# mgp25/OpenLTE

Measured on AMD Instinct MI355X. Metric: DL subframes/sec @20MHz 100RB 64QAM, full chain FFT->CE->demap->rate-unmatch->turbo(REF)->CRC (SURVEY 8d W4), higher is better.
Workload: dtype i8 IQ in, f32 FFT/CE/equaliser, i8 soft bits, i16 path metrics (differences exact modulo 2^16); 1 GPU; W4 full DL chain: 20 MHz/100 RB/64QAM, 9 allocations per subframe (8x12 PRB TBS 3240 + 1x4 PRB TBS 1064), 65536 subframes per GPU, int8 IQ in HBM; subframes_per_gpu=65536, N_ant=1, CFI=2, channel_estimate_form=compact, decoder=REF (reference-faithful, bit-exact), unique_subframes=96, streams_per_gpu=1

## Files before the change

openlte_amd/csrc/ctx.cc:

```cpp
#include <cmath>

#include <chrono>
#include <cstdlib>

#include <algorithm>

#include "ctx.hpp"
#include "build_id.h"

#include <cstring>

#include "lte_tables.h"

extern "C" {

int mi_lte_version(void) { return MI_LTE_VERSION; }
const char *mi_lte_build_id(void) { return MI_LTE_BUILD_ID; }

int mi_lte_device_count(void)
{
    int n = 0;
    if (hipGetDeviceCount(&n) != hipSuccess) return 0;
    return n;
}

int mi_lte_ctx_create(int device, mi_lte_ctx **out)
{
    if (!out) return MI_LTE_ERR_INVALID_ARG;
    *out  = nullptr;
    int n = mi_lte_device_count();
    if (n <= 0 || device < 0 || device >= n) {
        fprintf(stderr, "mi_lte: no usable HIP device %d (found %d); this library has no CPU fallback\n", device, n);
        return MI_LTE_ERR_NO_DEVICE;
    }
    mi_lte_ctx *ctx = new mi_lte_ctx();
    ctx->device     = device;
    if (const char *e = getenv("MI_LTE_NO_MERGED_DECODE")) ctx->merged_decode = atoi(e) == 0;
    hipDeviceProp_t prop;
    if (hipSetDevice(device) != hipSuccess || hipGetDeviceProperties(&prop, device) != hipSuccess) {
        delete ctx;
        return MI_LTE_ERR_HIP;
    }
    ctx->dev_name = std::string(prop.name) + " (" + prop.gcnArchName + ")";
    if (std::strncmp(prop.gcnArchName, "gfx950", 6) != 0) {
        fprintf(stderr, "mi_lte: device %d is %s, but the kernels are built for gfx950 only\n", device, prop.gcnArchName);
        delete ctx;
        return MI_LTE_ERR_NO_DEVICE;
    }
    if (hipStreamCreateWithFlags(&ctx->stream, hipStreamNonBlocking) != hipSuccess || hipEventCreate(&ctx->ev0) != hipSuccess ||
        hipEventCreate(&ctx->ev1) != hipSuccess) {
        delete ctx;
        return MI_LTE_ERR_HIP;
    }
    *out = ctx;
    return MI_LTE_OK;
}

void mi_lte_ctx_destroy(mi_lte_ctx *ctx)
{
    if (!ctx) return;
    (void)hipSetDevice(ctx->device);
    (void)hipStreamSynchronize(ctx->stream);
    if (ctx->host_cache_free) ctx->host_cache_free(ctx);
    for (void *p : ctx->owned) (void)hipFree(p);
    for (hipEvent_t e : ctx->prof_pool) (void)hipEventDestroy(e);
    if (ctx->scratch) (void)hipFree(ctx->scratch);
    if (ctx->h_small) (void)hipHostFree(ctx->h_small);
    if (ctx->h_bounce) (void)hipHostFree(ctx->h_bounce);
    for (int k = 0; k < 2; k++)
        if (ctx->ev_bounce[k]) (void)hipEventDestroy(ctx->ev_bounce[k]);
    if (ctx->h_flag) (void)hipHostFree(ctx->h_flag);
    if (ctx->ev0) (void)hipEventDestroy(ctx->ev0);
    if (ctx->ev1) (void)hipEventDestroy(ctx->ev1);
    if (ctx->stream) (void)hipStreamDestroy(ctx->stream);
    delete ctx;
}

int mi_lte_set_turbo_small_batch(mi_lte_ctx *ctx, uint32_t n_cb_max)
{
    if (!ctx) return MI_LTE_ERR_INVALID_ARG;
    ctx->siso_small_max = n_cb_max;
    return MI_LTE_OK;
}

int mi_lte_set_turbo_merged(mi_lte_ctx *ctx, uint32_t on)
{
    if (!ctx) return MI_LTE_ERR_INVALID_ARG;
    ctx->merged_decode = on != 0;
    return MI_LTE_OK;
}
// ... 498 lines not shown
```

openlte_amd/csrc/ctx.hpp:

```cpp
#pragma once

#include <hip/hip_runtime.h>

#include <cstdint>
#include <cstdio>
#include <map>
#include <string>
#include <vector>

#include "../../include/mi_lte.h"

struct TurboTables {
    uint16_t *d_pi  = nullptr;
    uint16_t *d_inv = nullptr;
    uint16_t *d_inv2 = nullptr;
    uint32_t *d_pi_row = nullptr, *d_inv_row = nullptr;
};

struct RmTables {
    uint16_t *d_tabs = nullptr;
    uint32_t *d_nnn  = nullptr;
};

enum : uint32_t { MI_FFT_TWC_P2 = 0, MI_FFT_TWC_P3 = 32, MI_FFT_TWC_L2048 = 288, MI_FFT_TWC_L1024 = 1312, MI_FFT_TWC_L256 = 1824, MI_FFT_TWC_L128 = 1952,
                  MI_FFT_TWC_X2 = 2016, MI_FFT_TWC_X3 = 2048,
                  MI_FFT_TWC_TOTAL = 2560 };

constexpr uint32_t MI_CRC_TAB_BIAS = 8;

struct mi_lte_ctx {
    int                device = -1;
    hipStream_t        stream = nullptr;
    hipEvent_t         ev0 = nullptr, ev1 = nullptr;
    std::string        err;
    std::string        dev_name;
    std::string        last_kernels;
    double             copy_rates[3] = {0, 0, 0};
    void              *scratch       = nullptr;
    size_t             scratch_bytes = 0;
    uint32_t          *h_flag = nullptr, *d_flag = nullptr;
    uint32_t           flag_seq = 0;
    uint32_t *bcjr_early_buf = nullptr; size_t bcjr_early_cap = 0;
    struct { uint32_t *chg; uint32_t n_pairs, n_iter, n_cb; } bcjr_early = {nullptr, 0, 0, 0};
    bool               bcjr_block_lds_set = false;
    uint32_t           siso_small_max = 4096;
    bool               merged_decode = true;
    void              *h_small = nullptr, *d_small = nullptr;
    void              *h_bounce = nullptr, *d_bounce = nullptr;
    hipEvent_t         ev_bounce[2] = {nullptr, nullptr};
    bool               bounce_failed = false;
    std::map<uint64_t, TurboTables> turbo_tables;
    std::map<uint32_t, RmTables>    rm_tables;
    std::vector<void *> owned;

    uint32_t *d_gold_x1 = nullptr, *d_gold_x2b = nullptr;
    uint32_t  gold_words = 0;
    void     *d_pusch_shapes = nullptr;

    float2   *d_fft_tw  = nullptr;
    uint32_t *d_crc_tab = nullptr;
    float2   *d_prach_tab = nullptr;
    float2   *d_prach_tab4 = nullptr;

    bool                                   prof_on = false, prof_armed = false;
    std::vector<hipEvent_t>                prof_pool;
    size_t                                 prof_used = 0;
    std::vector<std::pair<const char *, size_t>> prof_recs;
    std::string                            prof_report;

    void *host_cache = nullptr;
    void (*host_cache_free)(mi_lte_ctx *) = nullptr;
};

void mi_prof_begin(mi_lte_ctx *ctx, const char *name);
void mi_prof_end(mi_lte_ctx *ctx);

#define MI_LAUNCH(ctx, name, kernel, grid, block, shmem, ...)                                         \
    do {                                                                                             \
        mi_prof_begin((ctx), (name));                                                                \
        hipLaunchKernelGGL(kernel, grid, block, shmem, (ctx)->stream, __VA_ARGS__);                  \
        mi_prof_end((ctx));                                                                          \
    } while (0)

#define MI_HIP_CHECK(ctx, call)                                                                      \
    do {                                                                                             \
        hipError_t e_ = (call);                                                                      \
        if (e_ != hipSuccess) {                                                                      \
            (ctx)->err = std::string(#call) + ": " + hipGetErrorString(e_);                          \
            return MI_LTE_ERR_HIP;                                                                   \
        }                                                                                            \
    } while (0)

#define MI_H2D(ctx, d, h, n) do { const int rc_ = mi_lte_memcpy_h2d((ctx), (d), (h), (n)); if (rc_ != MI_LTE_OK) return rc_; } while (0)
#define MI_D2H(ctx, h, d, n) do { const int rc_ = mi_lte_memcpy_d2h((ctx), (h), (d), (n)); if (rc_ != MI_LTE_OK) return rc_; } while (0)

template <typename F> struct OnFail {
    F    f;
    bool armed = true;
    ~OnFail() { if (armed) f(); }
// ... 53 lines not shown
```

openlte_amd/csrc/turbo.hip:

```cpp
#include <algorithm>
#include <cstring>
#include <type_traits>
#include <vector>

#include "plan_core.hpp"

namespace {

constexpr uint32_t RX_NULL_AS_INT = 10000;

__host__ __device__ inline uint32_t kpad64(uint32_t K) { return (K + 63u) & ~63u; }


__device__ __forceinline__ int sbyte(uint32_t w, int k) { return (int)__builtin_amdgcn_sbfe(w, 8 * k, 8); }

typedef __attribute__((address_space(3))) const uint8_t  lds_u8_t;
typedef __attribute__((address_space(3))) const int8_t   lds_i8_t;
typedef __attribute__((address_space(3))) const uint16_t lds_u16_t;
__device__ __forceinline__ uint32_t lds_u8(uint32_t addr) { return *(lds_u8_t *)(uintptr_t)addr; }
__device__ __forceinline__ int      lds_i8(uint32_t addr) { return *(lds_i8_t *)(uintptr_t)addr; }
__device__ __forceinline__ uint32_t lds_u16(uint32_t addr) { return *(lds_u16_t *)(uintptr_t)addr; }

typedef short v2s __attribute__((ext_vector_type(2)));
__device__ __forceinline__ v2s      as_v2s(uint32_t w) { return __builtin_bit_cast(v2s, w); }
__device__ __forceinline__ uint32_t as_u32(v2s v) { return __builtin_bit_cast(uint32_t, v); }
__device__ __forceinline__ v2s      even2(uint32_t w) { return (as_v2s(w) << 8) >> 8; }
__device__ __forceinline__ v2s      odd2(uint32_t w) { return as_v2s(w) >> 8; }
__device__ __forceinline__ uint32_t merge_bytes(v2s e, v2s o) { return __builtin_amdgcn_perm(as_u32(o), as_u32(e), 0x06020400u); }
__device__ __forceinline__ v2s      abs2(v2s a) { return __builtin_elementwise_max(a, (v2s)(0) - a); }
__device__ __forceinline__ uint32_t neg_mask(v2s d)
{
    uint32_t m;
    asm("v_pk_ashrrev_i16 %0, 15, %1 op_sel_hi:[0,1]" : "=v"(m) : "v"(as_u32(d)));
    return m;
}
__device__ __forceinline__ v2s bit_select(uint32_t m, v2s yes, v2s no) { return as_v2s((as_u32(yes) & m) | (as_u32(no) & ~m)); }
__device__ __forceinline__ v2s half_sum(v2s a, v2s b)
{
    uint32_t t = as_u32(a + b);
    asm("" : "+v"(t));
    return as_v2s(t) >> 1;
}

__device__ __forceinline__ int soft_xor(int a, int b)
{
    int mag = (abs(a) + abs(b)) >> 1;
    return ((a < 0) != (b < 0)) ? -mag : mag;
}


template <typename Op> __device__ __forceinline__ int wave_reduce_i(int v, Op op)
{
    v = op(v, __builtin_amdgcn_update_dpp(v, v, 0xB1, 0xF, 0xF, false));
    v = op(v, __builtin_amdgcn_update_dpp(v, v, 0x4E, 0xF, 0xF, false));
    v = op(v, __builtin_amdgcn_update_dpp(v, v, 0x141, 0xF, 0xF, false));
    v = op(v, __builtin_amdgcn_update_dpp(v, v, 0x140, 0xF, 0xF, false));
    return op(op(__builtin_amdgcn_readlane(v, 0), __builtin_amdgcn_readlane(v, 16)), op(__builtin_amdgcn_readlane(v, 32), __builtin_amdgcn_readlane(v, 48)));
}
__device__ __forceinline__ int      wave_max_i(int v) { return wave_reduce_i(v, [](int a, int b) { return max(a, b); }); }
__device__ __forceinline__ uint32_t wave_xor_u(uint32_t v) { return (uint32_t)wave_reduce_i((int)v, [](int a, int b) { return a ^ b; }); }
__device__ __forceinline__ float    wave_max_f(float v)
{
    return __int_as_float(wave_max_i(__float_as_int(v)));
}

__device__ __forceinline__ float block_max_abs_f(float v, float *red )
{
    v = wave_max_f(v);
    __syncthreads();
    if ((threadIdx.x & 63) == 0) red[threadIdx.x >> 6] = v;
    __syncthreads();
    float r = red[0];
    for (uint32_t w = 1; w < (blockDim.x >> 6); w++) r = fmaxf(r, red[w]);
    return r;
// ... 352 lines not shown
    __device__ __forceinline__ void load16_pk(uint32_t u, int nvalid, uint32_t (&vp)[3][8], uint32_t e_lds, bool in_lds) const
    {
        auto emit = [&](int x, const int (&acc)[16]) {
#pragma unroll
            for (int j = 0; j < 8; j++) vp[x][j] = __builtin_amdgcn_perm((uint32_t)acc[2 * j + 1], (uint32_t)acc[2 * j], 0x05040100u);
        };
        if (in_lds) gather16_staged(e_lds, u, nvalid, emit);
        else        gather16(e, u, nvalid, emit);
    }
    __device__ __forceinline__ bool window_ok() const { return Nnn + 48 <= e_cap; }
    __device__ __forceinline__ void gather_windowed_pk(uint32_t u, int nvalid, uint32_t (&vp)[3][8], int8_t *lds, uint32_t el) const
    {
        uint4 *l = reinterpret_cast<uint4 *>(lds);
        for (uint32_t base = 0; base < E; base += Nnn) {
            const uint32_t len = min(Nnn, E - base), shift = base & 15u, end = shift + len, nq = end >> 4, tail = end & 15u;
            const uint4   *gp = reinterpret_cast<const uint4 *>(e + (base - shift));
            RankWords rw;
            load_ranks(u, nvalid, rw);
            if (base) __syncthreads();
#pragma unroll 4
            for (uint32_t w = threadIdx.x; w < nq; w += blockDim.x) l[w] = gp[w];
            if (threadIdx.x == (nq & 63u)) {
                uint4 t = make_uint4(0, 0, 0, 0);
                if (tail) {
                    t = gp[nq];
                    uint32_t c[4] = {t.x, t.y, t.z, t.w};
#pragma unroll
                    for (uint32_t k = 0; k < 4; k++) {
                        const int keep = (int)tail - 4 * (int)k;
                        c[k] = keep >= 4 ? c[k] : keep <= 0 ? 0u : (c[k] & ((1u << (8 * keep)) - 1u));
                    }
                    t = make_uint4(c[0], c[1], c[2], c[3]);
                }
                l[nq] = t;
            }
            __syncthreads();
            if (nvalid > 0) {
#pragma unroll
                for (int x = 0; x < 3; x++) {
                    const uint32_t w[8] = {rw.raw[x][0].x, rw.raw[x][0].y, rw.raw[x][0].z, rw.raw[x][0].w, rw.raw[x][1].x, rw.raw[x][1].y, rw.raw[x][1].z, rw.raw[x][1].w};
                    int acc[16];
#pragma unroll
                    for (int k = 0; k < 16; k++) {
                        const uint32_t r = (k & 1) ? (w[k >> 1] >> 16) : (w[k >> 1] & 0xFFFFu);
                        acc[k] = lds_i8(el + shift + min(r, len));
                    }
#pragma unroll
                    for (int j = 0; j < 8; j++)
                        vp[x][j] = as_u32(as_v2s(vp[x][j]) + as_v2s(__builtin_amdgcn_perm((uint32_t)acc[2 * j + 1], (uint32_t)acc[2 * j], 0x05040100u)));
                }
            }
        }
    }
};
__device__ __forceinline__ void SrcRateUnmatch::seg(const_seg_fwd_t &sg)
{
    tabs = (const uint16_t *)sg.tabs; nnn = (const uint32_t *)sg.nnn; g.desc += sg.cb_base;
}
struct SrcRateUnmatchPk : SrcRateUnmatch { static constexpr bool kPacked = true; };

constexpr uint32_t QTAB_N = 4096;
constexpr uint32_t QTAB_HALF = 2048;
constexpr uint32_t MTAB_N = 256;
constexpr uint32_t PREP_RED_AT = 2 * MTAB_N, PREP_E_AT = PREP_RED_AT + 64, PREP_QTAB_AT = PREP_E_AT, PREP_Q0_AT = PREP_QTAB_AT + QTAB_N;
__host__ __device__ constexpr uint32_t prep_lds_bytes(uint32_t Kp, uint32_t e_cap) { return PREP_E_AT + (e_cap > QTAB_N + Kp ? e_cap : QTAB_N + Kp); }

__device__ __forceinline__ uint32_t pack4u(uint32_t b0, uint32_t b1, uint32_t b2, uint32_t b3) { return b0 | (b1 << 8) | (b2 << 16) | (b3 << 24); }
__device__ __forceinline__ uint32_t bias4(uint32_t w) { return w ^ 0x80808080u; }
template <int K4> __device__ __forceinline__ uint32_t abs_sum2(uint32_t wa_biased, uint32_t wb_biased)
{
    return __builtin_amdgcn_msad_u8(wb_biased, 0x80u << (8 * K4), __builtin_amdgcn_msad_u8(wa_biased, 0x80u << (8 * K4), 0u));
}
__device__ __forceinline__ void abs_sum16(const uint4 &A, const uint4 &B, uint32_t (&w)[16], uint32_t &wmax)
{
    const uint32_t a[4] = {bias4(A.x), bias4(A.y), bias4(A.z), bias4(A.w)}, b[4] = {bias4(B.x), bias4(B.y), bias4(B.z), bias4(B.w)};
#pragma unroll
    for (int j = 0; j < 4; j++) {
        w[4 * j]     = abs_sum2<0>(a[j], b[j]);
        w[4 * j + 1] = abs_sum2<1>(a[j], b[j]);
        w[4 * j + 2] = abs_sum2<2>(a[j], b[j]);
        w[4 * j + 3] = abs_sum2<3>(a[j], b[j]);
        wmax = max(max(wmax, w[4 * j]), max(w[4 * j + 1], max(w[4 * j + 2], w[4 * j + 3])));
    }
}
__device__ __forceinline__ uint4 lookup16(uint32_t base, const uint32_t (&w)[16])
{
    uint32_t o[4];
#pragma unroll
    for (int j = 0; j < 4; j++) o[j] = pack4u(lds_u8(base + w[4 * j]), lds_u8(base + w[4 * j + 1]), lds_u8(base + w[4 * j + 2]), lds_u8(base + w[4 * j + 3]));
    return make_uint4(o[0], o[1], o[2], o[3]);
}
__device__ __forceinline__ uint4 gather16_bytes(uint32_t base, const uint32_t (&idx)[16]) { return lookup16(base, idx); }

template <typename Src, int NSLOT, bool MULTI = false>
#ifndef PREP_WPE
#define PREP_WPE 6
#endif
#ifndef PREP_WPE_PK
#define PREP_WPE_PK 6
#endif
__global__ __launch_bounds__(384) __attribute__((amdgpu_waves_per_eu(Src::kPacked ? PREP_WPE_PK : PREP_WPE, 8))) void k_turbo_prep(Src src, uint32_t K_arg, uint32_t n_cb_arg,
                                                    const uint16_t *__restrict__ pi_arg, PrepOut out, MultiArgs ma)
{
    static_assert(NSLOT == 1, "one unit per thread (K <= 6144 -> at most 384 units)");
    uint32_t K = K_arg, n_cb = n_cb_arg, bidx = blockIdx.x;
    size_t   seg_off = 0;
    const uint16_t *__restrict__ pi = pi_arg;
    if constexpr (MULTI) {
        const_seg_t &sg = multi_seg(ma, blockIdx.x >> 9);
        K = sg.K; n_cb = sg.n_cb; pi = (const uint16_t *)sg.pi; bidx = blockIdx.x - sg.wg_cb; seg_off = sg.arr_off;
        src.e_cap = sg.e_cap;
        src.seg(sg);
    }
    extern __shared__ __attribute__((aligned(16))) int8_t sm[];
    const uint32_t cb = xcd_cb(bidx, n_cb), tile = cb >> 6, lane = cb & 63, Kp = kpad64(K), n_units = Kp >> 4;
    const size_t   tile_off = seg_off + (size_t)tile * Kp * 64;
    if (cb >= n_cb) {
        if (MULTI && cb < ((n_cb + 63u) & ~63u) && threadIdx.x < n_units)
#pragma unroll
            for (int a = 0; a < 6; a++) *reinterpret_cast<uint4 *>(out.arr[a] + unit_off(tile_off, lane, threadIdx.x)) = make_uint4(0, 0, 0, 0);
        return;
    }
    int8_t        *qtab = sm + PREP_QTAB_AT, *qc = qtab + QTAB_HALF, *mtab1 = sm, *mtab2 = mtab1 + MTAB_N, *e_lds = sm + PREP_E_AT;
    int8_t        *q0_lds = sm + PREP_Q0_AT;
    float         *red_f  = reinterpret_cast<float *>(sm + PREP_RED_AT);
    int           *red_i  = reinterpret_cast<int *>(sm + PREP_RED_AT);
    src.init(cb, K);
    const uint32_t u  = threadIdx.x;
    const int      nv = (u < n_units) ? min(16, max(0, (int)K - 16 * (int)u)) : -1;
    const bool     e_in_lds = src.stage_e(e_lds);

    typedef typename std::conditional<Src::kIntPath, int, float>::type val_t;
    val_t    v[Src::kPacked ? 1 : 3][16];
    uint32_t vp[3][8];
    float    mx;
    int      mxi = 0;
    if constexpr (Src::kPacked) {
#pragma unroll
        for (int x = 0; x < 3; x++)
#pragma unroll
            for (int j = 0; j < 8; j++) vp[x][j] = 0;
        if (!e_in_lds && src.window_ok()) src.gather_windowed_pk(u, nv, vp, e_lds, PREP_E_AT);
        else if (nv > 0) src.load16_pk(u, nv, vp, PREP_E_AT, e_in_lds);
        v2s hi = (v2s)(0), lo = (v2s)(0);
#pragma unroll
        for (int x = 0; x < 3; x++)
#pragma unroll
            for (int j = 0; j < 8; j++) { hi = __builtin_elementwise_max(hi, as_v2s(vp[x][j])); lo = __builtin_elementwise_min(lo, as_v2s(vp[x][j])); }
        mxi = block_max_i(max(max((int)hi.x, (int)hi.y), -min((int)lo.x, (int)lo.y)), red_i);
        mx  = (float)mxi;
    } else {
        if (nv > 0) src.load16(u, nv, v, PREP_E_AT, e_in_lds);
        else {
#pragma unroll
            for (int x = 0; x < 3; x++)
#pragma unroll
                for (int k = 0; k < 16; k++) v[Src::kPacked ? 0 : x][k] = 0;
        }
        if constexpr (Src::kIntPath) {
            int hi = 0, lo = 0;
#pragma unroll
            for (int x = 0; x < 3; x++)
#pragma unroll
                for (int k = 0; k < 16; k += 2) { hi = max(max(hi, v[Src::kPacked ? 0 : x][k]), v[x][k + 1]); lo = min(min(lo, v[Src::kPacked ? 0 : x][k]), v[x][k + 1]); }
            mxi = block_max_i(max(hi, -lo), red_i);
            mx  = (float)mxi;
        } else {
            float mxv = 0;
#pragma unroll
            for (int x = 0; x < 3; x++)
#pragma unroll
                for (int k = 0; k < 16; k++) mxv = fmaxf(mxv, fabsf(v[Src::kPacked ? 0 : x][k]));
            mx = block_max_abs_f(mxv, red_f);
        }
    }
    const bool use_qtab = Src::kIntegerValued && mx < (float)QTAB_HALF;
    const bool identity = Src::kIntPath && mxi == 127;
    const bool halving = Src::kPacked && mxi == 254;
    if (use_qtab && !identity && !halving) {
        if constexpr (Src::kIntPath) {
            for (int d = (int)threadIdx.x - mxi; d <= mxi; d += (int)blockDim.x) qc[d] = (int8_t)(int)((float)d * 127.0f / mx);
        } else {
            for (uint32_t a = threadIdx.x; a <= (uint32_t)mx; a += blockDim.x) qtab[a] = (int8_t)(int)((float)a * 127.0f / mx);
        }
        __syncthreads();
    }

    uint4 Q[3];
#pragma unroll
    for (int x = 0; x < 3; x++) {
        if constexpr (Src::kPacked) {
            uint32_t o[4];
            if (identity) {
#pragma unroll
                for (int j = 0; j < 4; j++) o[j] = __builtin_amdgcn_perm(vp[x][2 * j + 1], vp[x][2 * j], 0x06040200u);
            } else if (halving) {
#pragma unroll
                for (int j = 0; j < 4; j++) {
                    const v2s a = as_v2s(vp[x][2 * j]), b = as_v2s(vp[x][2 * j + 1]);
                    o[j] = __builtin_amdgcn_perm(as_u32((b - (b >> 15)) >> 1), as_u32((a - (a >> 15)) >> 1), 0x06040200u);
                }
            } else {
                int d[16];
#pragma unroll
                for (int j = 0; j < 8; j++) { d[2 * j] = (int)__builtin_amdgcn_sbfe(vp[x][j], 0, 16); d[2 * j + 1] = (int)vp[x][j] >> 16; }
                if (use_qtab) {
#pragma unroll
                    for (int j = 0; j < 4; j++)
                        o[j] = pack4u(lds_u8(PREP_QTAB_AT + QTAB_HALF + d[4 * j]), lds_u8(PREP_QTAB_AT + QTAB_HALF + d[4 * j + 1]), lds_u8(PREP_QTAB_AT + QTAB_HALF + d[4 * j + 2]), lds_u8(PREP_QTAB_AT + QTAB_HALF + d[4 * j + 3]));
                } else {
                    int q[16];
#pragma unroll
                    for (int k = 0; k < 16; k++) q[k] = (int)((float)d[k] * 127.0f / mx);
                    const uint4 t = pack16(q);
                    o[0] = t.x; o[1] = t.y; o[2] = t.z; o[3] = t.w;
                }
            }
            Q[x] = make_uint4(o[0], o[1], o[2], o[3]);
        } else if (Src::kIntPath && identity) {
            int q[16];
#pragma unroll
            for (int k = 0; k < 16; k++) q[k] = (int)v[Src::kPacked ? 0 : x][k];
            Q[x] = pack16(q);
        } else if (Src::kIntPath && use_qtab) {
            uint32_t o[4];
#pragma unroll
            for (int j = 0; j < 4; j++)
                o[j] = pack4u(lds_u8(PREP_QTAB_AT + QTAB_HALF + v[Src::kPacked ? 0 : x][4 * j]), lds_u8(PREP_QTAB_AT + QTAB_HALF + v[Src::kPacked ? 0 : x][4 * j + 1]), lds_u8(PREP_QTAB_AT + QTAB_HALF + v[Src::kPacked ? 0 : x][4 * j + 2]), lds_u8(PREP_QTAB_AT + QTAB_HALF + v[Src::kPacked ? 0 : x][4 * j + 3]));
            Q[x] = make_uint4(o[0], o[1], o[2], o[3]);
        } else {
            int q[16];
            if (use_qtab) {
#pragma unroll
                for (int k = 0; k < 16; k++) {
                    const float f = v[Src::kPacked ? 0 : x][k];
                    const int   t = qtab[(int)fabsf(f)];
                    q[k]          = f < 0.0f ? -t : t;
                }
            } else {
#pragma unroll
                for (int k = 0; k < 16; k++) q[k] = (int)((float)v[Src::kPacked ? 0 : x][k] * 127.0f / mx);
            }
            Q[x] = pack16(q);
        }
        if (nv >= 0) *reinterpret_cast<uint4 *>(out.arr[x] + unit_off(tile_off, lane, u)) = Q[x];
    }
    if (nv >= 0) *reinterpret_cast<uint4 *>(q0_lds + 16 * u) = Q[0];
    __syncthreads();

    uint4 I0 = make_uint4(0, 0, 0, 0);
    if (nv > 0) {
        uint32_t idx[16];
        if constexpr (MULTI)
            load_idx16_at(reinterpret_cast<const_u32x4_t *>(reinterpret_cast<uintptr_t>(pi + 16 * (size_t)u)), nv, idx, K);
        else
            load_idx16(pi, u, nv, idx, K);
        I0 = gather16_bytes(PREP_Q0_AT, idx);
    }
    if (nv >= 0) *reinterpret_cast<uint4 *>(out.arr[3] + unit_off(tile_off, lane, u)) = I0;
    if (identity && src.hard_inputs()) {
        auto cnt4 = [](uint32_t a, uint32_t b) { return (a & 0x01010101u) + (b & 0x01010101u); };
        const uint32_t c1[4] = {cnt4(Q[1].x, Q[0].x), cnt4(Q[1].y, Q[0].y), cnt4(Q[1].z, Q[0].z), cnt4(Q[1].w, Q[0].w)};
        const uint32_t c2[4] = {cnt4(Q[2].x, I0.x), cnt4(Q[2].y, I0.y), cnt4(Q[2].z, I0.z), cnt4(Q[2].w, I0.w)};
        const uint32_t o1 = c1[0] | c1[1] | c1[2] | c1[3], o2 = c2[0] | c2[1] | c2[2] | c2[3];
        int w1max = (o1 & 0x02020202u) ? 254 : (o1 ? 127 : 0), w2max = (o2 & 0x02020202u) ? 254 : (o2 ? 127 : 0);
        block_max_i2(w1max, w2max, red_i);
        if (w1max != 0 && w2max != 0) {
            auto mag4 = [](uint32_t cnt, int W) { return W == 254 ? (cnt << 6) - ((cnt | (cnt >> 1)) & 0x01010101u) : (cnt << 7) - cnt; };
            if (nv >= 0) {
                *reinterpret_cast<uint4 *>(out.arr[4] + unit_off(tile_off, lane, u)) = make_uint4(mag4(c1[0], w1max), mag4(c1[1], w1max), mag4(c1[2], w1max), mag4(c1[3], w1max));
                *reinterpret_cast<uint4 *>(out.arr[5] + unit_off(tile_off, lane, u)) = make_uint4(mag4(c2[0], w2max), mag4(c2[1], w2max), mag4(c2[2], w2max), mag4(c2[3], w2max));
            }
            return;
        }
    }
    uint32_t w1[16], w2[16], w1m = 0, w2m = 0;
    abs_sum16(Q[1], Q[0], w1, w1m);
    abs_sum16(Q[2], I0, w2, w2m);
    int w1max = (int)w1m, w2max = (int)w2m;
    block_max_i2(w1max, w2max, red_i);
    auto closed = [](int W) { return W == 254 || W == 127; };
    auto closed16 = [](const uint32_t (&w)[16], int W) {
        uint32_t o[4];
#pragma unroll
        for (int j = 0; j < 4; j++) {
            const uint32_t p = pack4u(w[4 * j], w[4 * j + 1], w[4 * j + 2], w[4 * j + 3]);
            o[j] = W == 254 ? (p >> 1) & 0x7F7F7F7Fu : p;
        }
        return make_uint4(o[0], o[1], o[2], o[3]);
    };
    if (!(closed(w1max) && closed(w2max))) {
        const float W1 = (float)w1max, W2 = (float)w2max;
        for (uint32_t t = threadIdx.x; t < MTAB_N; t += blockDim.x) {
            const float w = (float)t;
            mtab1[t] = (int8_t)(int)(127.0f * (w / W1));
            mtab2[t] = (int8_t)(int)(127.0f * (w / W2));
        }
        __syncthreads();
    }
    if (nv >= 0) {
        *reinterpret_cast<uint4 *>(out.arr[4] + unit_off(tile_off, lane, u)) = closed(w1max) ? closed16(w1, w1max) : lookup16(0, w1);
// ... 1013 lines not shown
    MI_LAUNCH(ctx, "k_turbo_vote", (k_turbo_vote<GROUP, 1>), dim3(8 * xcd_chunk(n_cb)), dim3(cb_threads), 3 * Kp + 64, sc.va, K, n_cb, tb.d_inv2, d_c_bits, gd, MultiArgs{});
    MI_HIP_CHECK(ctx, hipGetLastError());
    ctx->last_kernels = "k_turbo_prep:1,k_turbo_siso:2,k_turbo_perm:1,k_turbo_vote:1";
    return MI_LTE_OK;
}

template <typename T>
static int turbo_ref_batch(mi_lte_ctx *ctx, const T *d_soft, uint32_t K, uint32_t n_cb, uint8_t *d_c_bits)
{
    SrcDirect<T> src{0, d_soft, nullptr};
    GroupDesc    none{};
    return turbo_ref_run<SrcDirect<T>, false>(ctx, src, K, n_cb, d_c_bits, none);
}

static int rm_rank_tables(mi_lte_ctx *ctx, uint32_t K, RmTables *out)
{
    auto it = ctx->rm_tables.find(K);
    if (it == ctx->rm_tables.end()) {
        RmTables t;
        MI_HIP_CHECK(ctx, hipMalloc((void **)&t.d_tabs, sizeof(uint16_t) * 12 * 3 * K));
        MI_HIP_CHECK(ctx, hipMalloc((void **)&t.d_nnn, sizeof(uint32_t) * 12));
        ctx->owned.push_back(t.d_tabs);
        ctx->owned.push_back(t.d_nnn);
        MI_LAUNCH(ctx, "k_rm_rank_table", k_rm_rank_table, dim3((3 * K + 255) / 256, 12), dim3(256), 0, K, t.d_tabs, t.d_nnn);
        MI_HIP_CHECK(ctx, hipGetLastError());
        it = ctx->rm_tables.emplace(K, t).first;
    }
    *out = it->second;
    return MI_LTE_OK;
}

static GroupDesc group_desc(const mi_lte_ctx *ctx, const MiDecodeIO &io, uint32_t cb_base = 0)
{
    return {io.d_allocs, io.d_cb_alloc + cb_base, io.d_e, io.d_e_off, io.d_e_len, io.d_out_bits, io.out_stride, io.d_status, ctx->d_crc_tab, io.ul ? 1u : 0u, io.packed ? 1u : 0u};
}
static uint32_t stage_cap(uint32_t e_max_bytes) { return (e_max_bytes + 16u + 63u) & ~63u; }

static bool mi_turbo_ref_multi_takes(uint32_t K, uint32_t e_max_bytes) { return (e_max_bytes + (3 * K - 81) - 1) / (3 * K - 81) <= 258; }

static int mi_turbo_ref_group(mi_lte_ctx *ctx, const MiKGroup &gr, const MiDecodeIO &io)
{
    int rc = mi_ctx_crc_table(ctx);
    if (rc != MI_LTE_OK) return rc;
    const GroupDesc gd = group_desc(ctx, io, gr.cb_base);
    RmTables rt;
    rc = rm_rank_tables(ctx, gr.K, &rt);
    if (rc != MI_LTE_OK) return rc;
    SrcRateUnmatch src;
    src.g    = gd;
    src.tabs = rt.d_tabs;
    src.nnn  = rt.d_nnn;
    const uint32_t cap = stage_cap(gr.e_max);
    src.e_cap          = (prep_lds_bytes(kpad64(gr.K), cap) <= 48 * 1024) ? cap : 0;
    if (mi_turbo_ref_multi_takes(gr.K, gr.e_max)) {
        SrcRateUnmatchPk pk;
        static_cast<SrcRateUnmatch &>(pk) = src;
        return turbo_ref_run<SrcRateUnmatchPk, true>(ctx, pk, gr.K, gr.n_cb, nullptr, gd, src.e_cap);
    }
    return turbo_ref_run<SrcRateUnmatch, true>(ctx, src, gr.K, gr.n_cb, nullptr, gd, src.e_cap);
}

static int mi_turbo_ref_multi(mi_lte_ctx *ctx, const MiKGroup *groups, uint32_t n_groups, const MiDecodeIO &io, MiMultiCache *cache)
{
    if (!groups || n_groups == 0 || n_groups > 0xFFFF || !cache) return MI_LTE_ERR_INVALID_ARG;
    int rc = mi_ctx_crc_table(ctx);
    if (rc != MI_LTE_OK) return rc;
    static const bool lds_ok = no_static_lds((const void *)k_turbo_prep<SrcRateUnmatchPk, 1, true>) && no_static_lds((const void *)k_turbo_perm<1, true>) &&
                               no_static_lds((const void *)k_turbo_vote<true, 1, true>);
    if (!lds_ok) { ctx->err = "turbo kernels were built with static LDS: absolute LDS addressing is invalid"; return MI_LTE_ERR_HIP; }
    constexpr int NCLS = 6;
    auto cls_of = [](uint32_t K) { return (int)((((kpad64(K) >> 4) + 63) >> 6) - 1); };
    const bool same = cache->built_for.size() == n_groups && memcmp(cache->built_for.data(), groups, sizeof(MiKGroup) * n_groups) == 0;
    if (!same) {
        cache->built_for.clear();
        std::vector<KSeg>     segs(n_groups);
        std::vector<uint32_t> map;
        MiMultiGeom          &G = cache->geom;
        G = MiMultiGeom{};
        uint64_t arr = 0;
        uint32_t cbs = 0;
        for (uint32_t i = 0; i < n_groups; i++) {
            const MiKGroup &gr = groups[i];
            if ((i && gr.K <= groups[i - 1].K) || gr.n_cb == 0) { ctx->err = "merged decode: groups must be non-empty and in ascending block size"; return MI_LTE_ERR_INVALID_ARG; }
            TurboTables tb;
            RmTables    rt;
            if ((rc = mi_ctx_turbo_tables(ctx, gr.K, 0, &tb)) != MI_LTE_OK || (rc = rm_rank_tables(ctx, gr.K, &rt)) != MI_LTE_OK) return rc;
            KSeg &sg = segs[i];
            memset(&sg, 0, sizeof(sg));
            const uint32_t Kp = kpad64(gr.K), cap = stage_cap(gr.e_max);
            sg.K = gr.K; sg.n_cb = gr.n_cb; sg.cb_base = gr.cb_base; sg.n_tiles = (gr.n_cb + 63) / 64;
            const uint32_t cap_w = (uint32_t)((15 * (size_t)(gr.K + 4) / 4 + 64 + 63) & ~(size_t)63);
            sg.e_cap = (prep_lds_bytes(Kp, cap) <= 48 * 1024) ? (Kp <= 1024 ? std::min(cap, cap_w) : cap) : cap_w;
            sg.arr_off = arr;
            typedef __attribute__((address_space(1))) const uint16_t gl16_t;
            typedef __attribute__((address_space(1))) const uint32_t gl32_t;
            sg.pi = (gl16_t *)tb.d_pi; sg.inv2 = (gl16_t *)tb.d_inv2; sg.tabs = (gl16_t *)rt.d_tabs; sg.nnn = (gl32_t *)rt.d_nnn;
            arr += (uint64_t)sg.n_tiles * Kp * 64;
            cbs = std::max(cbs, gr.cb_base + gr.n_cb);
            const int c = cls_of(gr.K);
            G.one_size[c] = (G.lds_prep[c] == 0 && gr.n_cb % 64 == 0) ? (int)i : -1;
            G.off_one[c] = sg.arr_off; G.e_cap_one[c] = sg.e_cap;
            G.lds_prep[c] = std::max(G.lds_prep[c], prep_lds_bytes(Kp, sg.e_cap));
            G.kp_max[c]   = std::max(G.kp_max[c], Kp);
        }
        G.arr_bytes = arr;
        G.n_slots   = cbs;
// ... 51 lines not shown
            *n_out = 4 * n_wg;
        };
        deal(G.n_wv1, &G.ord_wv1, &G.n_ord1);
        deal(G.n_wv23, &G.ord_wv23, &G.n_ord23);
        uint32_t tot = 0, kp_all = 0;
        for (uint32_t i = 0; i < n_groups; i++) { tot += groups[i].n_cb; kp_all = std::max(kp_all, kpad64(groups[i].K)); }
        G.gpw1 = gpw_of(tot); G.gpw23 = gpw_of(2 * tot); G.kp_all = kp_all;
        G.map_ws1 = (uint32_t)map.size();
        uint32_t wg = 0;
        for (uint32_t i = 0; i < n_groups; i++) {
            const uint32_t n = (groups[i].n_cb + G.gpw1 - 1) / G.gpw1;
            segs[i].ws1 = wg;
            map.insert(map.end(), n, i);
            wg += n;
        }
        G.n_ws1   = wg;
        G.map_ws23 = (uint32_t)map.size();
        wg = 0;
        for (uint32_t i = 0; i < n_groups; i++) {
            const uint32_t n = (2 * groups[i].n_cb + G.gpw23 - 1) / G.gpw23;
            segs[i].ws23 = wg;
            map.insert(map.end(), n, i);
            wg += n;
        }
        G.n_ws23 = wg;
        const size_t seg_bytes = sizeof(KSeg) * n_groups, map_bytes = (sizeof(uint32_t) * map.size() + 15) & ~(size_t)15, need = seg_bytes + map_bytes;
        if (need > cache->cap) {
            MI_HIP_CHECK(ctx, hipStreamSynchronize(ctx->stream));
            if (cache->d_tab) (void)hipFree(cache->d_tab);
            cache->d_tab = nullptr; cache->cap = 0;
            MI_HIP_CHECK(ctx, hipMalloc(&cache->d_tab, need + need / 4));
            cache->cap = need + need / 4;
        }
        std::vector<uint8_t> blob(need, 0);
        memcpy(blob.data(), segs.data(), seg_bytes);
        memcpy(blob.data() + seg_bytes, map.data(), sizeof(uint32_t) * map.size());
        MI_H2D(ctx, cache->d_tab, blob.data(), need);
        G.map_off = seg_bytes;
        cache->built_for.assign(groups, groups + n_groups);
    }
    const MiMultiGeom &G = cache->geom;
    const size_t A = G.arr_bytes;
    rc = mi_ctx_reserve_scratch(ctx, N_BYTE_ARRAYS * A + 3 * (A / 2) + (size_t)((G.n_slots + 63) & ~63u) * sizeof(CbDesc));
    if (rc != MI_LTE_OK) return rc;
    const RefScratch sc(ctx->scratch, A);
    const KSeg     *d_segs = (const KSeg *)cache->d_tab;
    const uint32_t *d_map  = (const uint32_t *)((const uint8_t *)cache->d_tab + G.map_off);

    GroupDesc gd = group_desc(ctx, io);
    gd.desc = sc.d_desc;
    MI_LAUNCH(ctx, "k_cb_desc", k_cb_desc_multi, dim3((G.n_slots + 255) / 256), dim3(256), 0, gd, G.n_slots, d_segs, n_groups, sc.d_desc);
    SrcRateUnmatchPk src;
    src.g = gd; src.tabs = nullptr; src.nnn = nullptr; src.e_cap = 0;
    for (int c = 0; c < NCLS; c++)
        if (G.grid_cb[c]) {
            if (G.one_size[c] >= 0) {
                const MiKGroup &gr = groups[G.one_size[c]];
                TurboTables tb;
                RmTables    rt;
                if ((rc = mi_ctx_turbo_tables(ctx, gr.K, 0, &tb)) != MI_LTE_OK || (rc = rm_rank_tables(ctx, gr.K, &rt)) != MI_LTE_OK) return rc;
                SrcRateUnmatchPk s1 = src;
                s1.tabs = rt.d_tabs; s1.nnn = rt.d_nnn; s1.g.desc = sc.d_desc + gr.cb_base; s1.e_cap = G.e_cap_one[c];
                PrepOut p1 = sc.po;
                for (int a = 0; a < 6; a++) p1.arr[a] += G.off_one[c];
                MI_LAUNCH(ctx, "k_turbo_prep", (k_turbo_prep<SrcRateUnmatchPk, 1, false>), dim3(G.grid_cb[c]), dim3(64 * (c + 1)), G.lds_prep[c], s1, gr.K, gr.n_cb, (const uint16_t *)tb.d_pi,
                          p1, MultiArgs{});
                continue;
            }
            MI_LAUNCH(ctx, "k_turbo_prep", (k_turbo_prep<SrcRateUnmatchPk, 1, true>), dim3(G.grid_cb[c]), dim3(64 * (c + 1)), G.lds_prep[c], src, 0u, 0u, (const uint16_t *)nullptr, sc.po,
                      (MultiArgs{d_segs, d_map + G.map_cb[c]}));
        }
    const bool small = G.n_slots <= ctx->siso_small_max;
    auto lds_small = [&](uint32_t gpw) { return sizeof(uint32_t) * gpw * (64 * 4 * 2 + (G.kp_all >> 5) * 4); };
    if (small)
        MI_LAUNCH(ctx, "k_turbo_siso_small", k_turbo_siso_small<true>, dim3(G.n_ws1), dim3(64), lds_small(G.gpw1), sc.s1, 0u, 0u, 0u, G.gpw1, (MultiArgs{d_segs, d_map + G.map_ws1}));
    else
    MI_LAUNCH(ctx, "k_turbo_siso", k_turbo_siso<true>, dim3(G.n_ord1 ? G.n_ord1 / 4 : (G.n_wv1 + 3) / 4), dim3(256), G.siso_pad1, sc.s1, 0u, G.n_wv1, 0u, (MultiArgs{d_segs, d_map + G.map_wv1}),
              G.n_ord1 ? d_map + G.ord_wv1 : (const uint32_t *)nullptr);
    for (int c = 0; c < NCLS; c++)
        if (G.grid_perm[c])
            MI_LAUNCH(ctx, "k_turbo_perm", (k_turbo_perm<1, true>), dim3(G.grid_perm[c]), dim3(64 * (c + 1)), MTAB_N + G.kp_max[c] + 32, sc.pa, 0u, 0u, (const uint16_t *)nullptr,
                      (MultiArgs{d_segs, d_map + G.map_perm[c]}));
    if (small)
        MI_LAUNCH(ctx, "k_turbo_siso_small", k_turbo_siso_small<true>, dim3(G.n_ws23), dim3(64), lds_small(G.gpw23), sc.s23, 0u, 0u, 1u, G.gpw23, (MultiArgs{d_segs, d_map + G.map_ws23}));
    else
    MI_LAUNCH(ctx, "k_turbo_siso", k_turbo_siso<true>, dim3(G.n_ord23 ? G.n_ord23 / 4 : (G.n_wv23 + 3) / 4), dim3(256), G.siso_pad23, sc.s23, 0u, G.n_wv23, 1u, (MultiArgs{d_segs, d_map + G.map_wv23}),
              G.n_ord23 ? d_map + G.ord_wv23 : (const uint32_t *)nullptr);
    for (int c = 0; c < NCLS; c++)
        if (G.grid_cb[c])
            MI_LAUNCH(ctx, "k_turbo_vote", (k_turbo_vote<true, 1, true>), dim3(G.grid_cb[c]), dim3(64 * (c + 1)), 3 * G.kp_max[c] + 64, sc.va, 0u, 0u, (const uint16_t *)nullptr,
                      (uint8_t *)nullptr, gd, (MultiArgs{d_segs, d_map + G.map_cb[c]}));
    MI_HIP_CHECK(ctx, hipGetLastError());
    return MI_LTE_OK;
}

int mi_turbo_ref_dispatch(mi_lte_ctx *ctx, const MiKGroup *groups, uint32_t n_groups, const MiDecodeIO &io, MiMultiCache *cache)
{
    std::vector<MiKGroup> take;
    if (ctx->merged_decode)
        for (uint32_t i = 0; i < n_groups; i++)
            if (mi_turbo_ref_multi_takes(groups[i].K, groups[i].e_max)) take.push_back(groups[i]);
    const bool merged = take.size() >= 2;
    int        rc;
    if (merged && (rc = mi_turbo_ref_multi(ctx, take.data(), (uint32_t)take.size(), io, cache)) != MI_LTE_OK) return rc;
    for (uint32_t i = 0; i < n_groups; i++) {
        const MiKGroup &gr = groups[i];
// ... 94 lines not shown
```

Before: 2.715 million subframes/s.

## Gather rate-unmatched soft bits column-wise from LDS with word loads and byte permutes

Adds a column-oriented rate-unmatch path for the packed turbo prep kernel. When the received soft bits are staged in LDS, each lane now detects progressive index runs and fetches 4 bytes per run with aligned word loads and alignbyte, instead of gathering one byte at a time. It then transposes the bytes with perm instructions and routes the outputs back through LDS using wave-level fences. The old bytewise path stays available behind an environment variable; the new path adds extra LDS round-trips and code complexity.

Result: slower. 2.673 million subframes/s (-1.6%).

```diff
diff --git a/openlte_amd/csrc/ctx.cc b/openlte_amd/csrc/ctx.cc
--- a/openlte_amd/csrc/ctx.cc
+++ b/openlte_amd/csrc/ctx.cc
@@ -36,6 +36,7 @@
     mi_lte_ctx *ctx = new mi_lte_ctx();
     ctx->device     = device;
     if (const char *e = getenv("MI_LTE_NO_MERGED_DECODE")) ctx->merged_decode = atoi(e) == 0;
+    if (const char *e = getenv("MI_LTE_BYTEWISE_UNMATCH")) ctx->rm_bytewise = atoi(e) != 0;
     hipDeviceProp_t prop;
     if (hipSetDevice(device) != hipSuccess || hipGetDeviceProperties(&prop, device) != hipSuccess) {
         delete ctx;
diff --git a/openlte_amd/csrc/ctx.hpp b/openlte_amd/csrc/ctx.hpp
--- a/openlte_amd/csrc/ctx.hpp
+++ b/openlte_amd/csrc/ctx.hpp
@@ -45,6 +45,7 @@
     bool               bcjr_block_lds_set = false;
     uint32_t           siso_small_max = 4096;
     bool               merged_decode = true;
+    bool               rm_bytewise = false;
     void              *h_small = nullptr, *d_small = nullptr;
     void              *h_bounce = nullptr, *d_bounce = nullptr;
     hipEvent_t         ev_bounce[2] = {nullptr, nullptr};
diff --git a/openlte_amd/csrc/turbo.hip b/openlte_amd/csrc/turbo.hip
--- a/openlte_amd/csrc/turbo.hip
+++ b/openlte_amd/csrc/turbo.hip
@@ -20,6 +20,12 @@
 __device__ __forceinline__ uint32_t lds_u8(uint32_t addr) { return *(lds_u8_t *)(uintptr_t)addr; }
 __device__ __forceinline__ int      lds_i8(uint32_t addr) { return *(lds_i8_t *)(uintptr_t)addr; }
 __device__ __forceinline__ uint32_t lds_u16(uint32_t addr) { return *(lds_u16_t *)(uintptr_t)addr; }
+
+__device__ __forceinline__ void wave_lds_fence()
+{
+    __builtin_amdgcn_fence(__ATOMIC_ACQ_REL, "wavefront");
+    __builtin_amdgcn_wave_barrier();
+}
 
 typedef short v2s __attribute__((ext_vector_type(2)));
 __device__ __forceinline__ v2s      as_v2s(uint32_t w) { return __builtin_bit_cast(v2s, w); }
@@ -478,6 +484,84 @@
             }
         }
     }
+
+    uint32_t bytewise = 0;
+    __device__ __forceinline__ static uint32_t lds_u32(uint32_t addr) { return *(__attribute__((address_space(3))) const uint32_t *)(uintptr_t)addr; }
+    template <int STEP> __device__ __forceinline__ static void fetch_run(uint32_t addr, uint32_t &w0, uint32_t &w1)
+    {
+        const uint32_t a = addr & ~3u, d0 = lds_u32(a), d1 = lds_u32(a + 4);
+        w0 = __builtin_amdgcn_alignbyte(d1, d0, addr);
+        if (STEP == 2) w1 = __builtin_amdgcn_alignbyte(lds_u32(a + 8), d1, addr);
+    }
+    __device__ __forceinline__ uint32_t column_bytes(uint32_t f, uint32_t step, bool prog, const uint16_t *tp, uint32_t nrow, uint32_t base, uint32_t el) const
+    {
+        if (f + base >= E) return 0u;
+        uint32_t r[4] = {f, f + step, f + 2 * step, f + 3 * step};
+        if (!prog) {
+#pragma unroll
+            for (uint32_t j = 1; j < 4; j++) r[j] = j < nrow ? (uint32_t)tp[32 * j] : 0xFFFFu;
+        }
+        uint32_t b[4];
+#pragma unroll
+        for (uint32_t j = 0; j < 4; j++) b[j] = lds_u8(el + min(r[j] + base, E));
+        return b[0] | (b[1] << 8) | (b[2] << 16) | (b[3] << 24);
+    }
+    __device__ __forceinline__ void load_cols_pk(uint32_t t, uint32_t (&vp)[3][8], uint32_t el) const
+    {
+        const uint32_t i0 = 128 * (t >> 3) + 4 * (t & 7);
+        if (i0 >= K_) return;
+        const uint32_t nrow = min(4u, (K_ - i0 + 31) >> 5);
+        uint2 fr[3], lr[3];
+#pragma unroll
+        for (int x = 0; x < 3; x++) {
+            const uint16_t *tp = tab + (size_t)x * K_ + i0;
+            fr[x] = *reinterpret_cast<const uint2 *>(tp);
+            lr[x] = *reinterpret_cast<const uint2 *>(tp + 32 * (nrow - 1));
+        }
+#pragma unroll
+        for (int x = 0; x < 3; x++) {
+            constexpr uint32_t SEL_LO = 0x05010400u, SEL_HI = 0x07030602u;
+            const uint32_t step = x ? 2u : 1u, span = step * (nrow - 1);
+            const uint32_t f[4] = {fr[x].x & 0xFFFFu, fr[x].x >> 16, fr[x].y & 0xFFFFu, fr[x].y >> 16};
+            const uint32_t l[4] = {lr[x].x & 0xFFFFu, lr[x].x >> 16, lr[x].y & 0xFFFFu, lr[x].y >> 16};
+            bool prog[4], fast[4];
+#pragma unroll
+            for (int m = 0; m < 4; m++) { prog[m] = l[m] - f[m] == span; fast[m] = prog[m] && l[m] < E; }
+            const uint32_t fmin = min(min(f[0], f[1]), min(f[2], f[3]));
+            const uint16_t *tp = tab + (size_t)x * K_ + i0;
+            for (uint32_t base = 0; base < E; base += Nnn) {
+                if (base && !__any(fmin + base < E)) break;
+                uint32_t c[4];
+                if (base == 0) {
+#pragma unroll
+                    for (int m = 0; m < 4; m++) {
+                        uint32_t w0, w1 = 0;
+                        if (x == 0) fetch_run<1>(el + (fast[m] ? f[m] : 0u), w0, w1);
+                        else        fetch_run<2>(el + (fast[m] ? f[m] : 0u), w0, w1);
+                        c[m] = x == 0 ? w0 : __builtin_amdgcn_perm(w1, w0, 0x06040200u);
+                    }
+                }
+                if (base || !(fast[0] && fast[1] && fast[2] && fast[3])) {
+#pragma unroll
+                    for (int m = 0; m < 4; m++)
+                        if (base || !fast[m]) c[m] = column_bytes(f[m], step, prog[m], tp + m, nrow, base, el);
+                }
+                const uint32_t ta01 = __builtin_amdgcn_perm(c[1], c[0], SEL_LO), tb01 = __builtin_amdgcn_perm(c[1], c[0], SEL_HI);
+                const uint32_t ta23 = __builtin_amdgcn_perm(c[3], c[2], SEL_LO), tb23 = __builtin_amdgcn_perm(c[3], c[2], SEL_HI);
+                uint32_t row[4] = {__builtin_amdgcn_perm(ta23, ta01, SEL_LO), __builtin_amdgcn_perm(ta23, ta01, SEL_HI),
+                                   __builtin_amdgcn_perm(tb23, tb01, SEL_LO), __builtin_amdgcn_perm(tb23, tb01, SEL_HI)};
+                if (nrow < 4) {
+#pragma unroll
+                    for (uint32_t j = 1; j < 4; j++) row[j] = j < nrow ? row[j] : 0u;
+                }
+#pragma unroll
+                for (int j = 0; j < 4; j++) {
+                    vp[x][2 * j]     = as_u32(as_v2s(vp[x][2 * j]) + even2(row[j]));
+                    vp[x][2 * j + 1] = as_u32(as_v2s(vp[x][2 * j + 1]) + odd2(row[j]));
+                }
+            }
+        }
+    }
 };
 __device__ __forceinline__ void SrcRateUnmatch::seg(const_seg_fwd_t &sg)
 {
@@ -561,12 +645,15 @@
     uint32_t vp[3][8];
     float    mx;
     int      mxi = 0;
+    bool cols = false;
+    if constexpr (Src::kPacked) cols = e_in_lds && !src.bytewise;
     if constexpr (Src::kPacked) {
 #pragma unroll
         for (int x = 0; x < 3; x++)
 #pragma unroll
             for (int j = 0; j < 8; j++) vp[x][j] = 0;
-        if (!e_in_lds && src.window_ok()) src.gather_windowed_pk(u, nv, vp, e_lds, PREP_E_AT);
+        if (cols) src.load_cols_pk(u, vp, PREP_E_AT);
+        else if (!e_in_lds && src.window_ok()) src.gather_windowed_pk(u, nv, vp, e_lds, PREP_E_AT);
         else if (nv > 0) src.load16_pk(u, nv, vp, PREP_E_AT, e_in_lds);
         v2s hi = (v2s)(0), lo = (v2s)(0);
 #pragma unroll
@@ -669,10 +756,32 @@
             }
             Q[x] = pack16(q);
         }
-        if (nv >= 0) *reinterpret_cast<uint4 *>(out.arr[x] + unit_off(tile_off, lane, u)) = Q[x];
-    }
-    if (nv >= 0) *reinterpret_cast<uint4 *>(q0_lds + 16 * u) = Q[0];
+        if (!cols && nv >= 0) *reinterpret_cast<uint4 *>(out.arr[x] + unit_off(tile_off, lane, u)) = Q[x];
+    }
+    if (cols) {
+        const uint32_t i0 = 128 * (u >> 3) + 4 * (u & 7);
+#pragma unroll
+        for (int xx = 0; xx < 3; xx++) {
+            const int      x    = (xx + 1) % 3;
+            const uint32_t w[4] = {Q[x].x, Q[x].y, Q[x].z, Q[x].w};
+#pragma unroll
+            for (uint32_t j = 0; j < 4; j++)
+                if (i0 + 32 * j < Kp) *reinterpret_cast<uint32_t *>(q0_lds + i0 + 32 * j) = w[j];
+            if (x != 0) {
+                wave_lds_fence();
+                if (nv >= 0) {
+                    Q[x] = *reinterpret_cast<const uint4 *>(q0_lds + 16 * u);
+                    *reinterpret_cast<uint4 *>(out.arr[x] + unit_off(tile_off, lane, u)) = Q[x];
+                } else Q[x] = make_uint4(0, 0, 0, 0);
+                wave_lds_fence();
+            }
+        }
+    } else if (nv >= 0) *reinterpret_cast<uint4 *>(q0_lds + 16 * u) = Q[0];
     __syncthreads();
+    if (cols && nv >= 0) {
+        Q[0] = *reinterpret_cast<const uint4 *>(q0_lds + 16 * u);
+        *reinterpret_cast<uint4 *>(out.arr[0] + unit_off(tile_off, lane, u)) = Q[0];
+    } else if (cols) Q[0] = make_uint4(0, 0, 0, 0);
 
     uint4 I0 = make_uint4(0, 0, 0, 0);
     if (nv > 0) {
@@ -1792,6 +1901,7 @@
     src.nnn  = rt.d_nnn;
     const uint32_t cap = stage_cap(gr.e_max);
     src.e_cap          = (prep_lds_bytes(kpad64(gr.K), cap) <= 48 * 1024) ? cap : 0;
+    src.bytewise       = ctx->rm_bytewise ? 1u : 0u;
     if (mi_turbo_ref_multi_takes(gr.K, gr.e_max)) {
         SrcRateUnmatchPk pk;
         static_cast<SrcRateUnmatch &>(pk) = src;
@@ -1949,6 +2059,7 @@
     MI_LAUNCH(ctx, "k_cb_desc", k_cb_desc_multi, dim3((G.n_slots + 255) / 256), dim3(256), 0, gd, G.n_slots, d_segs, n_groups, sc.d_desc);
     SrcRateUnmatchPk src;
     src.g = gd; src.tabs = nullptr; src.nnn = nullptr; src.e_cap = 0;
+    src.bytewise = ctx->rm_bytewise ? 1u : 0u;
     for (int c = 0; c < NCLS; c++)
         if (G.grid_cb[c]) {
             if (G.one_size[c] >= 0) {
```
